# volivan239/raytracing-course-hw

Measured on AMD Instinct MI355X. Metric: Msamples/sec at 1920x1080x256spp, higher is better.
Workload: dtype f32; 1 GPU; synth_room_v1_1920x1080x256; scene=synth_room_v1 (seed 20241223), triangles=268816, emissive_triangles=4204, width=1920, height=1080, spp=256, ray_depth=6, parallelism=pixel tiles 32x32 round-robin over 1 GPU(s), bvh_nodes=265605, bvh_depth=24, light_bvh_depth=19, device_bytes=120573816

## Files before the change

raytracing-course-hw_amd/csrc/device/rt_device.h:

```cpp
#pragma once
#include <hip/hip_runtime.h>
#include "rt_types.h"

#define RT_DEV __device__ __forceinline__

namespace rtamd {
namespace dev {

struct F3 { float x, y, z; };
RT_DEV F3 f3(float x, float y, float z) { F3 r; r.x = x; r.y = y; r.z = z; return r; }
RT_DEV F3 f3(const float *p) { return f3(p[0], p[1], p[2]); }
RT_DEV F3 operator+(F3 a, F3 b) { return f3(a.x + b.x, a.y + b.y, a.z + b.z); }
RT_DEV F3 operator-(F3 a, F3 b) { return f3(a.x - b.x, a.y - b.y, a.z - b.z); }
RT_DEV F3 operator*(F3 a, F3 b) { return f3(a.x * b.x, a.y * b.y, a.z * b.z); }
RT_DEV F3 operator*(float k, F3 p) { return f3(k * p.x, k * p.y, k * p.z); }
RT_DEV F3 neg(F3 a) { return f3(-a.x, -a.y, -a.z); }
RT_DEV float dot(F3 a, F3 b) { return a.x * b.x + a.y * b.y + a.z * b.z; }
RT_DEV F3 crossr(F3 a, F3 o) { return f3(a.z * o.y - a.y * o.z, a.x * o.z - a.z * o.x, a.y * o.x - a.x * o.y); }
RT_DEV float len2(F3 a) { return dot(a, a); }
RT_DEV float len(F3 a) { return sqrtf(len2(a)); }
RT_DEV F3 normalize(F3 a) { return (1.0f / len(a)) * a; }
RT_DEV float smin(float a, float b) { return (b < a) ? b : a; }
RT_DEV float smax(float a, float b) { return (a < b) ? b : a; }

// ... 202 lines not shown
    F3 ro = o - a;
    float dn = dot(d, n);
    t = -dot(ro, n) / dn;
    if (!(t > 0 && t < RT_T_MAX)) return false;
    inside = dn > 0;
    F3 p = ro + t * d;
    float c1 = RT_MAGIC1_0 * p.x + RT_MAGIC1_1 * p.y + RT_MAGIC1_2 * p.z;
    float c2 = RT_MAGIC2_0 * p.x + RT_MAGIC2_1 * p.y + RT_MAGIC2_2 * p.z;
    float yy = (c1 * T.a2 - c2 * T.a1) / T.den;
    float xx = T.a2 == 0 ? (c1 - T.b1 * yy) / T.a1 : (c2 - T.b2 * yy) / T.a2;
    u = xx; v = yy;
    if (u < 0 || v < 0 || u + v > 1) return false;
    return true;
}

RT_DEV bool tri_test_closer(const TriIsect &T, F3 o, F3 d, float keep_t, float &t, float &u, float &v, bool &inside) {
    F3 a = f3(T.ax, T.ay, T.az), n = f3(T.nx, T.ny, T.nz);
    F3 ro = o - a;
    float dn = dot(d, n);
    t = -dot(ro, n) / dn;
    if (!(t > 0 && t < RT_T_MAX)) return false;
    if (t > keep_t) return false;
    inside = dn > 0;
    F3 p = ro + t * d;
    float c1 = RT_MAGIC1_0 * p.x + RT_MAGIC1_1 * p.y + RT_MAGIC1_2 * p.z;
    float c2 = RT_MAGIC2_0 * p.x + RT_MAGIC2_1 * p.y + RT_MAGIC2_2 * p.z;
    float yy = (c1 * T.a2 - c2 * T.a1) / T.den;
    float xx = T.a2 == 0 ? (c1 - T.b1 * yy) / T.a1 : (c2 - T.b2 * yy) / T.a2;
    u = xx; v = yy;
    if (u < 0 || v < 0 || u + v > 1) return false;
    return true;
}

RT_DEV TriIsect load_isect(const TriIsect *p) {
    const float4 *q = reinterpret_cast<const float4 *>(p);
    float4 a = q[0], b = q[1], c = q[2];
    TriIsect T;
    T.ax = a.x; T.ay = a.y; T.az = a.z; T.nx = a.w;
    T.ny = b.x; T.nz = b.y; T.a1 = b.z; T.b1 = b.w;
    T.a2 = c.x; T.b2 = c.y; T.den = c.z; T.pad = __float_as_uint(c.w);
    return T;
}

struct RayInv { F3 o, inv; };
RT_DEV RayInv make_ray_inv(F3 o, F3 d) {
    RayInv r;
    r.o = o;
    float dx = fabsf(d.x) > 1e-30f ? d.x : copysignf(1e-30f, d.x);
    float dy = fabsf(d.y) > 1e-30f ? d.y : copysignf(1e-30f, d.y);
    float dz = fabsf(d.z) > 1e-30f ? d.z : copysignf(1e-30f, d.z);
    r.inv = f3(1.0f / dx, 1.0f / dy, 1.0f / dz);
    return r;
}
RT_DEV bool slab_test(float4 lo, float4 hi, const RayInv &r, float tbest, float &tnear) {
    float t0x = (lo.x - r.o.x) * r.inv.x, t1x = (hi.x - r.o.x) * r.inv.x;
    float t0y = (lo.y - r.o.y) * r.inv.y, t1y = (hi.y - r.o.y) * r.inv.y;
    float t0z = (lo.z - r.o.z) * r.inv.z, t1z = (hi.z - r.o.z) * r.inv.z;
    float tmin = fmaxf(fmaxf(fminf(t0x, t1x), fminf(t0y, t1y)), fminf(t0z, t1z));
    float tmax = fminf(fminf(fmaxf(t0x, t1x), fmaxf(t0y, t1y)), fmaxf(t0z, t1z));
    tmin = fmaf(-fabsf(tmin), 4.8e-7f, tmin);
    tmax = fmaf(fabsf(tmax), 4.8e-7f, tmax);
    tnear = tmin;
    return (tmin <= tmax) & (tmax >= 0.f) & (tmin <= tbest);
}

typedef float rt_f2 __attribute__((ext_vector_type(2)));
struct RayGrid { float cx, cy, cz, ix, iy, iz; uint32_t sx, sy, sz; };
RT_DEV RayGrid ray_grid_idle() {
    RayGrid g;
    g.cx = 0.f; g.cy = 0.f; g.cz = 0.f; g.ix = 1.f; g.iy = 1.f; g.iz = 1.f; g.sx = 0x03020100u; g.sy = 0x03020100u; g.sz = 0x03020100u;
    return g;
}
#define RT_GRID_RAY_IDLE ray_grid_idle()
RT_DEV RayGrid make_ray_grid(const NodeGrid &G, F3 o, F3 d) {
// ... 410 lines not shown
```

raytracing-course-hw_amd/csrc/device/rt_exact.h:

```cpp
#pragma once
#include "rt_kernels_hw8.h"

namespace rtamd {
namespace dev {

#define PT_SHADE_EXACT 4
#define WF_MISS 0xFFFFFFFFu
#define WF_INSIDE_BIT 0x40000000u
#define WF_GAP_SHIFT 24
#define WF_INDEX_MASK 0x00FFFFFFu
#define WF_SAMPLE_MASK 0x01FFFFFFu
#define WF_VERIFIED_BIT 0x80000000u

template <class A>
RT_DEV void ref_closest_hit(const SceneView &S, F3 o, F3 d, A &&stack, float &best_t, float &best_u, float &best_v, uint32_t &hit) {
    best_t = RT_T_MAX; best_u = 0.f; best_v = 0.f; hit = WF_MISS;
    if (S.n_tris == 0) return;
    RefBest best = {false, RT_T_MAX};
    ref_left_first<RT_STACK_SIZE>(S.ref_nodes, o, d, stack, best, [&](uint32_t first, uint32_t last) {
        for (uint32_t i = first; i < last; i++) {
            const TriIsect T = load_isect(S.tri_isect + i);
            float t, u, v; bool in;
            if (tri_test(T, o, d, t, u, v, in) && (!best.have || t < best.t)) {
                best.have = true; best.t = t; best_u = u; best_v = v; hit = i | (in ? WF_INSIDE_BIT : 0u);
// ... 85 lines not shown
    const float window = need - fminf(fminf(ax, ay), az);
    return worst >= need && exit_ >= need && tmax - t > window;
}

RT_DEV bool pt_tripwire(const SceneView &S, F3 o, F3 d) {
    if (S.n_tripwire_groups == 0u) return false;
    const float dx = fabsf(d.x) > 1e-30f ? d.x : copysignf(1e-30f, d.x), dy = fabsf(d.y) > 1e-30f ? d.y : copysignf(1e-30f, d.y), dz = fabsf(d.z) > 1e-30f ? d.z : copysignf(1e-30f, d.z);
    RayInv r; r.o = o; r.inv = f3(pt_rcp(dx), pt_rcp(dy), pt_rcp(dz));
    const float4 *rec = reinterpret_cast<const float4 *>(S.tripwires);
    bool pierced = false;
    for (uint32_t g = 0; g < S.n_tripwire_groups; g++) {
        const float4 lo = rec[2 * g], hi = rec[2 * g + 1];
        float tn;
        if (slab_test(lo, hi, r, RT_T_MAX, tn)) {
            const uint32_t first = __float_as_uint(lo.w), count = __float_as_uint(hi.w);
            for (uint32_t m = first; m < first + count; m++) {
                const float4 mlo = rec[2 * m];
                if (slab_test(mlo, rec[2 * m + 1], r, RT_T_MAX, tn)) {
                    const uint32_t fi = __float_as_uint(mlo.w);
                    const TriIsect T = load_isect(S.tri_isect + fi);
                    float t, u, v; bool inside;
                    if (tri_test(T, o, d, t, u, v, inside)) {
                        const float4 *bx = reinterpret_cast<const float4 *>(S.tri_box) + 2 * (size_t)fi;
                        const float4 blo = bx[0], bhi = bx[1];
                        if (!pt_deep_inside(f3(blo.x, blo.y, blo.z), f3(bhi.x, bhi.y, bhi.z), o + t * d, d, t, S.box_c2)) pierced = true;
                    }
                }
            }
        }
    }
    return pierced;
}

RT_DEV bool pt_light_test(const LightRec *L, F3 x, F3 d, bool &last, uint32_t &index, float &t, float &u, float &v, bool &inside) {
    const TriIsect T = load_isect(&L->isect);
    last = (T.pad & 1u) != 0;
    index = T.pad >> 1;
    return tri_test(T, x, d, t, u, v, inside);
}
RT_DEV float pt_light_pdf_hit(const SceneView &S, const LightRec *L, F3 x, F3 d, float t, float u, float v, bool inside, bool &robust) {
    robust = true;
    const float4 *q = reinterpret_cast<const float4 *>(L) + 3;
    float4 q1 = q[1], q2 = q[2], q3 = q[3];
    float point_prob = q1.z;
    F3 n3 = f3(q1.w, q2.x, q2.y), dn1 = f3(q2.z, q2.w, q3.x), dn2 = f3(q3.y, q3.z, q3.w);
    F3 sn = n3 + u * dn1 + v * dn2;
    sn = normalize(sn);
    if (inside) sn = neg(sn);
    if (S.hw7) { const TriIsect T = load_isect(&L->isect); F3 n = f3(T.nx, T.ny, T.nz); sn = normalize(inside ? neg(n) : n); }
    F3 y = x + t * d;
    if (S.exact_boxes == 1u) {
        const float4 blo = q[4], bhi = q[5];
        robust = pt_box_robust(f3(blo.x, blo.y, blo.z), f3(bhi.x, bhi.y, bhi.z), y, d, t, S.box_c2);
    }
    return point_prob * len2(x - y) / fabsf(dot(d, sn));
}
RT_DEV float pt_light_pdf_one(const SceneView &S, const LightRec *L, F3 x, F3 d, bool &last, bool &robust, uint32_t &index) {
    TriIsect T = load_isect(&L->isect);
    last = (T.pad & 1u) != 0;
    index = T.pad >> 1;
    robust = true;
    float t, u, v; bool inside;
    if (!tri_test(T, x, d, t, u, v, inside)) return 0.f;
    const float4 *q = reinterpret_cast<const float4 *>(L) + 3;
    float4 q1 = q[1], q2 = q[2], q3 = q[3];
    float point_prob = q1.z;
    F3 n3 = f3(q1.w, q2.x, q2.y), dn1 = f3(q2.z, q2.w, q3.x), dn2 = f3(q3.y, q3.z, q3.w);
    F3 sn = n3 + u * dn1 + v * dn2;
    sn = normalize(sn);
    if (inside) sn = neg(sn);
    if (S.hw7) { F3 n = f3(T.nx, T.ny, T.nz); sn = normalize(inside ? neg(n) : n); }
    F3 y = x + t * d;
    if (S.exact_boxes == 1u) {
        const float4 blo = q[4], bhi = q[5];
        robust = pt_box_robust(f3(blo.x, blo.y, blo.z), f3(bhi.x, bhi.y, bhi.z), y, d, t, S.box_c2);
    }
    return point_prob * len2(x - y) / fabsf(dot(d, sn));
}


}
}
```

raytracing-course-hw_amd/csrc/device/rt_persistent.h:

```cpp
#pragma once
#include "rt_path_source.h"
#include "rt_pt_queue.h"

namespace rtamd {
namespace dev {

#define P8_WAVES 4
#define P8_THREADS (64 * P8_WAVES)
#define P8_PER_CU 5
#define PT_MAX_PATHS 5120
#define PT_MIN_GROUP 16
#define PT_NW (PT_MAX_PATHS / 32)
#define PT_BIT_T 1u
#define PT_BIT_L 2u
#define PT_Q_TRACE 0
#define PT_Q_LIGHT 1
#define PT_Q_SHADE 2
#define PT_Q_XLIGHT 3
#define PT_Q_XTRACE 4
#define PT_N_LIVE 5
#define PT_W_TRACE 6
#define PT_W_LIGHT 7
#define PT_GSHIFT 15
#define PT_COST_TRACE_NODE 1u
#define PT_COST_TRACE_TRI 1u
#define PT_COST_LIGHT_NODE 2u
#define PT_COST_LIGHT_TEST 2u
#define PT_COST_SHADE 14u
#define PT_DEBUG_BLOCKS 2048
#define PT_DRAINED 0xFFFFFFFEu
#define PT_T_OVERFLOW (-1.f)
#define PT_WIDE_NONE 0
#define PT_WIDE_WENT 1
#define PT_WIDE_FULL 2
RT_DEV uint32_t pt_near_key(bool entered, uint32_t key) { return entered ? key : 0xFFFFFFFFu; }
RT_DEV void pt_order(uint32_t &ka, uint32_t &ca, uint32_t &kb, uint32_t &cb) {
    const bool s = kb < ka;
    const uint32_t k = s ? kb : ka, c = s ? cb : ca;
    kb = s ? ka : kb; cb = s ? ca : cb;
    ka = k; ca = c;
}
RT_DEV int pt_wide_step_nearest(const GpuNode4Q *nodes, const RayGrid &ray, float cull_t, uint32_t (*stack)[64], int lane, int &sp, int cap, uint32_t &cur) {
    const uint4 *q = reinterpret_cast<const uint4 *>(nodes + cur);
    const uint4 b0 = q[0], b1 = q[1], b2 = q[2], b3 = q[3];
    uint32_t k0, k1, k2, k3;
    const bool h0 = slab_enter_q(b0, ray, cull_t, k0), h1 = slab_enter_q(b1, ray, cull_t, k1);
    const bool h2 = slab_enter_q(b2, ray, cull_t, k2), h3 = slab_enter_q(b3, ray, cull_t, k3);
    k0 = pt_near_key(h0, k0); k1 = pt_near_key(h1, k1); k2 = pt_near_key(h2, k2); k3 = pt_near_key(h3, k3);
    uint32_t c0 = b0.w, c1 = b1.w, c2 = b2.w, c3 = b3.w;
    pt_order(k0, c0, k1, c1); pt_order(k2, c2, k3, c3); pt_order(k0, c0, k2, c2); pt_order(k1, c1, k3, c3); pt_order(k1, c1, k2, c2);
    const int nh = (int)h0 + (int)h1 + (int)h2 + (int)h3;
    if (nh == 0) return PT_WIDE_NONE;
    if (sp + nh - 1 > cap) return PT_WIDE_FULL;
    if (nh > 3) stack[sp++][lane] = c3;
    if (nh > 2) stack[sp++][lane] = c2;
    if (nh > 1) stack[sp++][lane] = c1;
    cur = c0;
    return PT_WIDE_WENT;
}
RT_DEV void pt_wide_enter_all(const GpuNode4Q *nodes, uint32_t cur, const RayGrid &ray, uint4 &b0, uint4 &b1, uint4 &b2, uint4 &b3,
                              bool &h0, bool &h1, bool &h2, bool &h3) {
    const uint4 *q = reinterpret_cast<const uint4 *>(nodes + cur);
    b0 = q[0]; b1 = q[1]; b2 = q[2]; b3 = q[3];
    h0 = slab_test_q(b0, ray); h1 = slab_test_q(b1, ray); h2 = slab_test_q(b2, ray); h3 = slab_test_q(b3, ray);
}
RT_DEV int pt_wide_step_all(const GpuNode4Q *nodes, const RayGrid &ray, uint32_t (*stack)[64], int lane, int &sp, int cap, uint32_t &cur) {
    uint4 b0, b1, b2, b3;
    bool h0, h1, h2, h3;
    pt_wide_enter_all(nodes, cur, ray, b0, b1, b2, b3, h0, h1, h2, h3);
    const int nh = (int)h0 + (int)h1 + (int)h2 + (int)h3;
    if (nh == 0) return PT_WIDE_NONE;
    if (sp + nh - 1 > cap) return PT_WIDE_FULL;
    const int first = h0 ? 0 : h1 ? 1 : h2 ? 2 : 3;
    if (h3 && first != 3) stack[sp++][lane] = b3.w;
    if (h2 && first < 2) stack[sp++][lane] = b2.w;
    if (h1 && first < 1) stack[sp++][lane] = b1.w;
    cur = first == 0 ? b0.w : first == 1 ? b1.w : first == 2 ? b2.w : b3.w;
    return PT_WIDE_WENT;
}
#define PT_LIGHT_SETTLE 1
template <int LEVELS>
RT_DEV int pt_light_reach(const SceneView &S, const RayGrid &ray, int &steps) {
    uint4 b[4];
    bool h[4];
    pt_wide_enter_all(S.light_walk_nodes4, 0u, ray, b[0], b[1], b[2], b[3], h[0], h[1], h[2], h[3]);
    steps = 1;
    if (!(h[0] | h[1] | h[2] | h[3])) return 0;
    if (LEVELS < 2) return 2;
    for (int c = 0; c < 4; c++) {
        if (!h[c]) continue;
        if (b[c].w & RT_LEAF_BIT) return 2;
        uint4 g0, g1, g2, g3;
        bool e0, e1, e2, e3;
        pt_wide_enter_all(S.light_walk_nodes4, b[c].w, ray, g0, g1, g2, g3, e0, e1, e2, e3);
        steps++;
        if (e0 | e1 | e2 | e3) return 2;
    }
    return 1;
}
#define PT_EXACT_BATCH 16

struct PtShared {
    uint32_t stack[P8_WAVES][P8_STACK][64];
    uint32_t need[5][PT_NW];
    uint32_t pending[PT_NW * 2];
    uint32_t groups[PT_MAX_PATHS / PT_MIN_GROUP];
    uint32_t cost[PT_MAX_PATHS / PT_MIN_GROUP];
    int cnt[16];
};
static_assert(PT_EXACT_BATCH * RT_STACK_SIZE <= P8_STACK * 64, "the exact role's stacks must fit the wave's LDS stack area");
static_assert(sizeof(PtShared) <= (128 / P8_PER_CU) * 1280, "P8_PER_CU workgroups per CU: the CU's 128 LDS granules of 1,280 bytes shared evenly");

struct PtParams {
    uint32_t n_groups;
    uint32_t group_shift;
    const uint32_t *group_ofs, *group_ids;
    uint32_t *group_cost;
    uint32_t resume;
    int refill, leaf_batch;
    int shade_min;
    int shade_thr0, shade_thr_step;
    int cost_t, cost_l;
    uint32_t front_first;
    int prio;
    unsigned long long deadline_ticks;
    unsigned long long *counters;
    unsigned long long *debug;
// ... 134 lines not shown
                if (went == PT_WIDE_NONE) {
                    if (sp != 0) cur = stack[--sp][lane];
                    else if (pend != RT_EMPTY_LEAF) cur = PT_DRAINED;
                    else end_walk();
                } else if (went == PT_WIDE_FULL) {
                    w.full();
                    pend = RT_EMPTY_LEAF; pend2 = RT_EMPTY_LEAF; pend3 = RT_EMPTY_LEAF;
                    end_walk();
                }
            }
        }
        clk.lap(prof.t_part[K][1]);
        const bool at_leaf = active && pend != RT_EMPTY_LEAF;
        if (COUNT) { prof.leaf_iters[K]++; prof.leaf_lane_iters[K] += __popcll(pt_ballot(at_leaf)); }
        if (at_leaf) {
            uint32_t i = pend & ~RT_LEAF_BIT, more = pend2, more2 = pend3;
            typename WK::Leaf lf;
            for (;;) {
                const bool last = w.test(i, sp, lf);
                if (COUNT) n_tris++;
                steps += WK::COST_TEST;
                if (!last) i++;
                else if (more == RT_EMPTY_LEAF) break;
                else { i = more & ~RT_LEAF_BIT; more = more2; more2 = RT_EMPTY_LEAF; }
            }
            const bool over = w.leaves_done(lf, sp);
            pend = RT_EMPTY_LEAF; pend2 = RT_EMPTY_LEAF; pend3 = RT_EMPTY_LEAF;
            if (cur == PT_DRAINED || over) end_walk();
        }
        clk.lap(prof.t_part[K][2]);
    }
}

template <class T> RT_DEV const T *pt_own_pointer(const T *p) { asm volatile("" : "+s"(p)); return p; }
struct PtTraceWalk {
    typedef PtTraceQueue Queue;
    static constexpr uint32_t COST_NODE = PT_COST_TRACE_NODE, COST_TEST = PT_COST_TRACE_TRI;
    const SceneView &S; const WfView &W; PtShared &sh; const PtParams &P; uint32_t (*stack)[64];
    const GpuNode4Q *nodes = pt_own_pointer(S.nodes4);
    const int lane = threadIdx.x & 63;
    F3 o = f3(0.f, 0.f, 0.f), d = f3(0.f, 0.f, 1.f);
    RayGrid ray = RT_GRID_RAY_IDLE;
    uint32_t hit = WF_MISS;
    float best_t = RT_T_MAX, best_u = 0.f, best_v = 0.f;
    float cull_t = RT_T_MAX, t2 = 2.f * RT_T_MAX, h_ray = 0.f;
    struct Leaf {};
    RT_DEV void begin(uint32_t slot) {
        const float4 *r = wf_rec(W, slot);
        float4 q0 = r[0], q1 = r[1];
        o = f3(q0.x, q0.y, q0.z); d = f3(q0.w, q1.x, q1.y);
        ray = make_ray_grid(S.grid, o, d);
        h_ray = S.exact_boxes ? pt_look_behind_abs(d, S.box_c2x) : 0.f;
        hit = WF_MISS; best_t = RT_T_MAX; cull_t = RT_T_MAX; t2 = 2.f * RT_T_MAX; best_u = 0.f; best_v = 0.f;
    }
    RT_DEV int step(uint32_t &cur, int &sp) { return pt_wide_step_nearest(nodes, ray, cull_t, stack, lane, sp, P8_STACK, cur); }
    RT_DEV void full() { best_t = PT_T_OVERFLOW; best_u = 0.f; best_v = 0.f; hit = 0u; t2 = PT_T_OVERFLOW; }
    RT_DEV bool test(uint32_t i, int, Leaf &) {
        TriIsect T = load_isect(S.tri_walk + i);
        float t, u, v; bool inside;
        const uint32_t fi = T.pad >> 1;
        if (tri_test_closer(T, o, d, cull_t, t, u, v, inside)) {
            const uint32_t best_i = hit & WF_INDEX_MASK;
            if (t < best_t || (t == best_t && fi < best_i)) {
                t2 = fminf(t2, best_t);
                best_t = t; best_u = u; best_v = v; hit = fi | (inside ? WF_INSIDE_BIT : 0u);
                cull_t = t + fmaxf(S.cull_k * t, h_ray);
            } else t2 = fminf(t2, t);
        }
        return (T.pad & 1u) != 0u;
    }
    RT_DEV bool leaves_done(Leaf &, int) { return false; }
    RT_DEV uint32_t end(uint32_t l, uint32_t slot, uint32_t steps) {
        wf_rec(W, slot)[2] = make_float4(best_t, best_u, best_v, __uint_as_float(S.exact_boxes && hit != WF_MISS ? hit | pt_gap_code(best_t, t2) : hit));
        pt_book_cost(sh, P, l, steps);
        return l;
    }
};

template <bool COUNT> struct PtLightWalk {
    typedef PtLightQueue<PT_Q_XLIGHT> Queue;
    static constexpr uint32_t COST_NODE = PT_COST_LIGHT_NODE, COST_TEST = PT_COST_LIGHT_TEST;
    const SceneView &S; const WfView &W; PtShared &sh; const PtParams &P; uint32_t (*stack)[64]; PtProf &prof;
    const GpuNode4Q *nodes = pt_own_pointer(S.light_walk_nodes4);
    const LightRec *lights = pt_own_pointer(S.lights_walk);
    const int lane = threadIdx.x & 63;
    bool overflow = false;
    int k = 0;
    F3 o = f3(0.f, 0.f, 0.f), d = f3(0.f, 0.f, 1.f);
    RayGrid ray = RT_GRID_RAY_IDLE;
    struct Leaf { bool held = false; uint32_t h_i = 0u, h_li = 0u; float h_t = 0.f, h_u = 0.f, h_v = 0.f; bool h_in = false; };
    RT_DEV void begin(uint32_t slot) {
        const float4 *r = wf_rec(W, slot);
        float4 q0 = r[0], q1 = r[1];
        o = f3(q0.x, q0.y, q0.z); d = f3(q0.w, q1.x, q1.y);
        ray = make_ray_grid(S.grid, o, d);
        k = 0; overflow = false;
    }
    RT_DEV int step(uint32_t &cur, int &sp) { return pt_wide_step_all(nodes, ray, stack, lane, sp, P8_STACK - 2 * k - 1, cur); }
    RT_DEV void full() { overflow = true; }
    RT_DEV void take(Leaf &lf, int sp) {
        bool robust;
        const float term = pt_light_pdf_hit(S, lights + lf.h_i, o, d, lf.h_t, lf.h_u, lf.h_v, lf.h_in, robust);
        if (COUNT && term != 0.f) prof.light_hits++;
        if (term != 0.f) {
            if (!robust || k >= WF_MAX_LIGHT_HITS || sp + 2 * k + 2 >= P8_STACK) overflow = true;
            else {
                int j = k;
                while (j > 0 && stack[P8_STACK - 1 - 2 * (j - 1)][lane] > lf.h_li) {
                    stack[P8_STACK - 1 - 2 * j][lane] = stack[P8_STACK - 1 - 2 * (j - 1)][lane];
                    stack[P8_STACK - 2 - 2 * j][lane] = stack[P8_STACK - 2 - 2 * (j - 1)][lane];
                    j--;
                }
                stack[P8_STACK - 1 - 2 * j][lane] = lf.h_li; stack[P8_STACK - 2 - 2 * j][lane] = __float_as_uint(term); k++;
            }
        }
        lf.held = false;
    }
    RT_DEV bool test(uint32_t i, int sp, Leaf &lf) {
        bool last, inside; uint32_t li; float t, u, v;
        if (COUNT) prof.light_tests++;
        if (pt_light_test(lights + i, o, d, last, li, t, u, v, inside)) {
            if (lf.held) take(lf, sp);
            lf.held = true; lf.h_i = i; lf.h_li = li; lf.h_t = t; lf.h_u = u; lf.h_v = v; lf.h_in = inside;
        }
        return last;
    }
    RT_DEV bool leaves_done(Leaf &lf, int sp) { if (lf.held) take(lf, sp); return false; }
    RT_DEV uint32_t end(uint32_t l, uint32_t slot, uint32_t steps) {
        pt_book_cost(sh, P, l, steps);
        if (overflow) return l | 0x80000000u;
        float v = 0.f;
        if (k == 1) v = __uint_as_float(stack[P8_STACK - 2][lane]);
        else if (k == 2) v = __uint_as_float(stack[P8_STACK - 2][lane]) + __uint_as_float(stack[P8_STACK - 4][lane]);
        else if (k > 2) {
            const uint32_t nl = S.n_lights;
            for (int j = 1; j < k; j++) {
                uint32_t a0 = stack[P8_STACK - 1 - 2 * (j - 1)][lane], b0 = stack[P8_STACK - 1 - 2 * j][lane];
                uint32_t len = b0 - a0;
                uint32_t lv = 31u - (uint32_t)__clz((int)len);
                uint16_t m0 = S.light_sep[(size_t)lv * nl + a0], m1 = S.light_sep[(size_t)lv * nl + (b0 - (1u << lv))];
                stack[j - 1][lane] = m0 < m1 ? m0 : m1;
            }
            for (int n = k; n > 1; n--) {
                int best = 1;
                uint32_t bd = stack[0][lane];
                for (int i = 2; i < n; i++) { uint32_t di = stack[i - 1][lane]; if (di > bd) { bd = di; best = i; } }
                float merged = __uint_as_float(stack[P8_STACK - 2 - 2 * (best - 1)][lane]) + __uint_as_float(stack[P8_STACK - 2 - 2 * best][lane]);
                stack[P8_STACK - 2 - 2 * (best - 1)][lane] = __float_as_uint(merged);
                for (int i = best; i < n - 1; i++) {
                    stack[P8_STACK - 2 - 2 * i][lane] = stack[P8_STACK - 2 - 2 * (i + 1)][lane];
                    stack[i - 1][lane] = stack[i][lane];
                }
            }
            v = __uint_as_float(stack[P8_STACK - 2][lane]);
// ... 366 lines not shown
                r[3] = make_float4(0.f, 0.f, 0.f, __uint_as_float(wf_pack(0, false, (uint32_t)R.samples)));
                if (P.counters && pt_source_counts(R, gslot)) atomicAdd(&P.counters[CNT_SRC_NO_PATH], 1ull);
                return false;
            }
        } else {
            if (R.sample_seeds) wf_sample_seed(R, rng, gslot, x, y, 0u);
            wf_camera_ray(S, R, rng, x, y, o, d);
        }
        r[0] = make_float4(o.x, o.y, o.z, d.x);
        r[1] = make_float4(d.y, d.z, __uint_as_float(rng.x), rng.saved);
        r[2] = make_float4(0.f, 0.f, 0.f, 0.f);
        r[3] = make_float4(sum.x, sum.y, sum.z, __uint_as_float(wf_pack(0, rng.has_saved, R.accum ? (uint32_t)R.sample_first : 0u)));
        return true;
    }
    RT_DEV uint32_t resumed_sample(uint32_t slot) { return (__float_as_uint(reinterpret_cast<const float *>(wf_rec(W, slot) + 3)[3]) >> 6) & WF_SAMPLE_MASK; }
    RT_DEV bool seed_wire(uint32_t slot) {
        if constexpr ((FEAT & WF_FEAT_SOURCE) != 0) {
            const float4 *nr = wf_rec(W, slot);
            const float4 n0 = nr[0], n1 = nr[1];
            return pt_source_exact(S, f3(n0.x, n0.y, n0.z), f3(n0.w, n1.x, n1.y));
        }
        if (!S.n_tripwire_groups) return false;
        const float4 *nr = wf_rec(W, slot);
        const float4 n0 = nr[0], n1 = nr[1];
        return pt_tripwire(S, f3(n0.x, n0.y, n0.z), f3(n0.w, n1.x, n1.y));
    }
    RT_DEV bool rare(PtWave &wv) {
        const bool queued = pt_count(&sh.cnt[PT_Q_XLIGHT]) + pt_count(&sh.cnt[PT_Q_XTRACE]) > 0;
        if (queued) pt_exact_batch(S, W, sh, wv, &stack[0][0], n_xlight, n_xtrace);
        return queued;
    }
    RT_DEV PtShaded shade(uint32_t got, uint32_t &n_light, unsigned long long &n_nodes, PtProf &prof) {
        const uint32_t lane = threadIdx.x & 63u;
        int todo = 0;
        bool discarded = false;
        if (COUNT && P.trace_buf && got != PT_NONE) {
            const uint32_t tslot = pt_slot(sh, got);
            int tx, ty; bool tin; size_t toi;
            wf_slot_to_pixel(R, tslot + W.slot_base, tx, ty, tin, toi);
            if (tin && ty * R.width + tx == P.trace_pixel) {
                const float4 *tr = wf_rec(W, tslot);
                const uint32_t k = atomicAdd(reinterpret_cast<uint32_t *>(P.trace_buf), 1u);
                if (4u * k + 5u <= P.trace_cap) for (int q = 0; q < 4; q++) P.trace_buf[1 + 4 * k + q] = tr[q];
            }
        }
        PtShadeLap<COUNT> lp;
        if (got != PT_NONE) { PtPark pk; pk.p = (PtLdsWord)&stack[0][lane]; todo = pt_shade_lean<FEAT>(S, R, W, pt_slot(sh, got), pk, discarded, lp); }
        if constexpr (COUNT) {
            for (int k = 0; k < 5; k++) {
                const unsigned long long m = pt_ballot(lp.d[k] != 0u);
                if (m) { prof.t_shade[k] += (uint32_t)__builtin_amdgcn_readlane((int)lp.d[k], __builtin_ctzll(m)); prof.shade_lanes[k] += __popcll(m); }
            }
            prof.shade_last += __popcll(pt_ballot(lp.last));
        }
        n_discarded += __popcll(pt_ballot(discarded));
        const bool next = got != PT_NONE && todo != PT_SHADE_EXACT && (todo & WF_NEXT_TRACE), with_light = next && (todo & WF_NEXT_LIGHT);
        bool wire = false;
        bool settled = false;
        int settle_steps = 0;
        if (next && (S.n_tripwire_groups || ((COUNT || PT_LIGHT_SETTLE) && with_light))) {
            const float4 *nr = wf_rec(W, pt_slot(sh, got));
            const float4 n0 = nr[0], n1 = nr[1];
            const F3 o = f3(n0.x, n0.y, n0.z), d = f3(n0.w, n1.x, n1.y);
            if (S.n_tripwire_groups) wire = pt_tripwire(S, o, d);
            if ((COUNT || PT_LIGHT_SETTLE) && with_light) {
                const int reach = pt_light_reach<COUNT ? 2 : PT_LIGHT_SETTLE>(S, make_ray_grid(S.grid, o, d), settle_steps);
                if (COUNT) { prof.light_reach[0] += reach == 0; prof.light_reach[1] += reach == 1; }
                settled = reach < PT_LIGHT_SETTLE;
                if (settled) {
                    const int depth = (int)(__float_as_uint(reinterpret_cast<const float *>(nr + 3)[3]) & 15u);
                    float *pdf = reinterpret_cast<float *>(wf_entry(W, pt_slot(sh, got), depth)) + 3;
                    *pdf = *pdf + 0.f / S.n_lights_f;
                }
            }
        }
        if constexpr ((FEAT & WF_FEAT_SOURCE) != 0) {
            if (next && !wire) {
                const float4 *nr = wf_rec(W, pt_slot(sh, got));
                if ((__float_as_uint(reinterpret_cast<const float *>(nr + 3)[3]) & (15u | WF_PENDING_BIT)) == 0u) {
                    const float4 n0 = nr[0], n1 = nr[1];
                    wire = pt_source_exact(S, f3(n0.x, n0.y, n0.z), f3(n0.w, n1.x, n1.y));
                }
            }
        }
        n_light += __popcll(pt_ballot(settled));
        if (COUNT && settled) n_nodes += (unsigned long long)settle_steps;
        PtShaded s;
        s.trace = next;
        s.light = with_light && !settled;
        s.xtrace = (got != PT_NONE && todo == PT_SHADE_EXACT) || wire;
        s.done = got != PT_NONE && (todo == 0 || todo == WF_PARKED);
        if (got != PT_NONE && todo != PT_SHADE_EXACT) s.cost = (uint32_t)PT_COST_SHADE + (settled ? PT_COST_LIGHT_NODE * (uint32_t)settle_steps : 0u);
        return s;
    }
    RT_DEV void flush(uint32_t lane, const PtProf &prof) {
        if (lane == 0) {
            if (n_discarded) atomicAdd(&P.counters[CNT_DISCARDED], (unsigned long long)n_discarded);
            if (n_xtrace) atomicAdd(&P.counters[CNT_EXACT_CLOSEST], (unsigned long long)n_xtrace);
            if (n_xlight) atomicAdd(&P.counters[CNT_EXACT_LIGHT], (unsigned long long)n_xlight);
        }
        if (!COUNT) return;
        atomicAdd(&P.counters[CNT_P8_LIGHT_HITS], prof.light_hits); atomicAdd(&P.counters[CNT_P8_LIGHT_TESTS], prof.light_tests);
        atomicAdd(&P.counters[CNT_P8_LIGHT_REACH], prof.light_reach[0]); atomicAdd(&P.counters[CNT_P8_LIGHT_REACH + 1], prof.light_reach[1]);
        if (lane == 0) {
            atomicAdd(&P.counters[CNT_P8_WALK_ITERS], prof.iters[0]); atomicAdd(&P.counters[CNT_P8_WALK_ITERS + 1], prof.lane_iters[0]);
            atomicAdd(&P.counters[CNT_P8_WALK_ITERS + 2], prof.iters[1]); atomicAdd(&P.counters[CNT_P8_WALK_ITERS + 3], prof.lane_iters[1]);
            atomicAdd(&P.counters[CNT_P8_STINTS], prof.stints); atomicAdd(&P.counters[CNT_P8_SHADE_BATCHES], prof.shade_batches); atomicAdd(&P.counters[CNT_P8_SHADE_ITEMS], prof.shade_items);
            for (int k = 0; k < 3; k++) atomicAdd(&P.counters[CNT_P8_HANDOFF_TIME + k], prof.t_sub[0][k]);
            atomicAdd(&P.counters[CNT_P8_HANDOFFS], prof.refills[0]);
            for (int k = 0; k < 5; k++) { atomicAdd(&P.counters[CNT_P8_SHADE_TIME + k], prof.t_shade[k]); atomicAdd(&P.counters[CNT_P8_SHADE_LANES + k], prof.shade_lanes[k]); }
            atomicAdd(&P.counters[CNT_P8_SHADE_LAST], prof.shade_last);
// ... 22 lines not shown
```

raytracing-course-hw_amd/csrc/device/rt_types.h:

```cpp
#pragma once
#include <stdint.h>

namespace rtamd {

#define RT_MAX_DEPTH 16
#define RT_STACK_SIZE 64
#define P8_STACK 24

enum CounterSlot {
    CNT_CLOSEST = 0,
    CNT_LIGHT = 1,
    CNT_NODE_VISITS = 2,
    CNT_TRI_TESTS = 3,
    CNT_WF_NODE_ITERS = 4,
    CNT_WF_LEAF_PHASES = 5,
    CNT_WF_LEAF_LANES = 6,
    CNT_WF_REFILLS = 7,
    CNT_WF_LANE_NODES = 8,
    CNT_WF_LANE_TRIS = 9,
    CNT_DISCARDED = 10,
    CNT_WF_SLOW_LIGHT = 11,
    CNT_P6_EXACT_LIGHT = 11,
    CNT_EXACT_CLOSEST = 12,
    CNT_EXACT_LIGHT = 13,
// ... 39 lines not shown
#define RT_GRID_BORDER 4
struct NodeGrid { float lo[3], step[3], istep[3]; };

struct TriIsect {
    float ax, ay, az;
    float nx, ny, nz;
    float a1, b1;
    float a2, b2;
    float den;
    uint32_t pad;
};
static_assert(sizeof(TriIsect) == 48, "TriIsect must be 48 bytes");

struct TriShade {
    float n3[3], dn1[3], dn2[3];
    float t3[3], dt1[3], dt2[3];
    float uv3[2], duv1[2], duv2[2];
    float tanw;
    uint32_t material;
    uint32_t orig;
    uint32_t pad;
};
static_assert(sizeof(TriShade) == 112, "TriShade must be 112 bytes");

struct LightRec {
    TriIsect isect;
    float b[3], c[3];
    float point_prob;
    float n3[3], dn1[3], dn2[3];
    float box_lo[3], pad0;
    float box_hi[3], pad1;
};
static_assert(sizeof(LightRec) == 48 + 64 + 32, "LightRec must be 144 bytes");

struct GpuRefNode {
    float mn[3]; uint32_t left;
    float mx[3]; uint32_t right;
    uint32_t first, last, pad0, pad1;
};
static_assert(sizeof(GpuRefNode) == 48, "GpuRefNode must be 48 bytes");

struct GpuMaterial {
    float base_color[3]; float metallic_factor;
    float emission[3];   float roughness_factor;
    int32_t base_color_tex, emissive_tex, metallic_roughness_tex, normal_tex;
};
static_assert(sizeof(GpuMaterial) == 48, "GpuMaterial must be 48 bytes");

struct GpuImage {
    uint64_t offset;
    int32_t width, height;
};

struct SceneView {
    const GpuNode *nodes;
    const TriIsect *tri_isect;
    float cull_k;
    const TriIsect *tri_walk;
    const TriShade *tri_shade;
    const GpuNode *light_nodes;
    const LightRec *lights;
    const GpuNode *light_walk_nodes;
    const float *tripwires;
    uint32_t n_tripwire_groups;
    const GpuNode4Q *nodes4, *light_walk_nodes4;
    NodeGrid grid;
    const LightRec *lights_walk;
    const uint16_t *light_sep;
    const GpuMaterial *materials;
    const GpuImage *images;
    const uint8_t *texels;
    const float *srgb_lut;
    const GpuRefNode *ref_nodes, *ref_light_nodes;
    const float *tri_box;
    float box_c2;
    float box_c2x;
    uint32_t exact_boxes;
    uint32_t n_tris, n_lights, n_components;
    float n_lights_f, n_components_f;
    uint32_t n_nodes;
    uint32_t last_level_emission_only;
    uint32_t hw7;
    int32_t env_image;
    float cam_pos[3], cam_right[3], cam_up[3], cam_fwd[3];
    float bg[3];
    float tan_fov_y;
};

struct RenderView {
    int32_t width, height, samples, ray_depth;
    int32_t sample_stop;
    int32_t tile_w, tile_h, tiles_x, tiles_y;
    int32_t shard_index, shard_count;
    uint32_t n_shard_tiles;
    float tan_fov_x;
    float inv_samples;
    float *out_rgb;
    uint8_t *out_rgb8;
    uint32_t *work_counter;
    unsigned long long *counters;
// ... 18 lines not shown
```

raytracing-course-hw_amd/csrc/rtamd_scene.hip:

```cpp
#include <hip/hip_runtime.h>
#include <cmath>
#include <cstdio>
#include <cstdlib>
#include <cstring>
#include <memory>
#include <string>
#include <vector>
#include "../../include/rtamd.h"
#include "host/host_scene.h"
#include "host/png.h"
#include "host/scene_prep.h"
#include "host/shared_prep.h"
#include "host/device_build.h"
#include "host/knobs.h"
#include "host/rt_scene.h"
#include "device/rt_node_grid.h"

namespace rtamd {
static thread_local std::string g_last_error;
void set_error(const std::string &msg) { g_last_error = msg; }
}
using namespace rtamd;

namespace {
// ... 183 lines not shown
        const uint32_t n = desc->n_triangles;
        uint64_t scratch = 0;
        OwnedDev d_walk_box;
        if (!P.walk_box.empty()) d_walk_box.p = upload(P.walk_box, scratch);
        const DeviceTree t = build_leaf_ordered(s.get(), d_walk_box.p ? (const float *)d_walk_box.p : V.tri_box, V.tri_isect, n, P.box_pad, P8_STACK,
                                                11, true, V.tri_walk);
        V.nodes = t.nodes;
        up.bytes += (uint64_t)t.n_nodes * sizeof(GpuNode) + (uint64_t)n * sizeof(TriIsect);
        bvh_depth = t.depth;
        n_nodes = t.n_nodes;
        s->info.bvh_build_ms = t.build_ms; s->info.bvh_on_device = 1;
    } else {
        V.nodes = up(P.nodes);
        V.tri_walk = V.tri_isect;
    }
    if (P.bvh_depth > RT_STACK_SIZE - 2)
        return fail(RT_ERR_LIMIT, "the reference's scene BVH is deeper than the exact walk's stack (" + std::to_string(P.bvh_depth) + ")");
    if (bvh_depth > RT_STACK_SIZE - 2 || P.light_bvh_depth > RT_STACK_SIZE - 2)
        return fail(RT_ERR_LIMIT, "scene BVH deeper than the kernel's traversal stack (" + std::to_string(bvh_depth) + "/" +
                                      std::to_string(P.light_bvh_depth) + ")");
    V.light_nodes = up(P.light_nodes);
    V.light_sep = up(P.light_sep);
    upload_ref_trees(V, P, up);
    set_triangle_view(V, *desc, P, 2u);
    V.box_c2x *= (float)env_float("RTAMD_C2X_SCALE", 1.0);
    V.exact_boxes = (env_flag("RTAMD_NO_EXACT_BOXES") || fast_build) ? 0u : 1u;
    if (env_flag("RTAMD_DIAG_LOOKBEHIND_ONLY")) V.exact_boxes = 2u;
    V.n_tripwire_groups = (V.exact_boxes != 1u || env_flag("RTAMD_NO_TRIPWIRES")) ? 0u : P.n_tripwire_groups;
    V.tripwires = V.n_tripwire_groups ? up(P.tripwires) : nullptr;
    V.lights = up(P.lights);
    uint32_t n_light_walk_nodes = 0;
    {
        const uint32_t nl = (uint32_t)P.lights.size();
        std::vector<LightRec> tagged = P.lights;
        for (uint32_t i = 0; i < nl; i++) tagged[i].isect.pad = (i << 1) | (tagged[i].isect.pad ? 1u : 0u);
        if (nl >= 64 && !env_flag("RTAMD_HOST_LIGHT_BVH")) {
            uint64_t scratch = 0;
            OwnedDev d_tagged(upload(tagged, up.bytes));
            OwnedDev d_lbox(upload(P.light_walk_box, scratch));
            const DeviceTree lt = build_leaf_ordered(s.get(), (const float *)d_lbox.p, (const LightRec *)d_tagged.p, nl, P.box_pad, 16,
                                                     11, true, V.lights_walk);
            V.light_walk_nodes = lt.nodes;
            up.bytes += (uint64_t)lt.n_nodes * sizeof(GpuNode);
            s->light_walk_depth = lt.depth;
            n_light_walk_nodes = lt.n_nodes;
        } else {
            V.light_walk_nodes = V.light_nodes;
            n_light_walk_nodes = (uint32_t)P.light_nodes.size();
            V.lights_walk = up(tagged);
            s->light_walk_depth = P.light_bvh_depth;
        }
    }
    V.materials = up(P.materials);
    V.images = up(P.images);
    V.texels = up(P.texels);
    V.srgb_lut = up(std::vector<float>(P.srgb_lut, P.srgb_lut + 256));
    V.n_nodes = n_nodes;
    V.last_level_emission_only = 1;
    for (uint32_t i = 0; i < desc->n_materials; i++) {
        const rt_material &m = desc->materials[i];
        if (!(m.metallic_factor >= 0 && m.metallic_factor <= 1 && m.base_color[0] >= 0 && m.base_color[1] >= 0 && m.base_color[2] >= 0))
            V.last_level_emission_only = 0;
    }
    if (env_flag("RTAMD_NO_LAST_LEVEL_SHORTCUT")) V.last_level_emission_only = 0;
    V.env_image = P.env_image;
    make_walk_nodes(s.get(), V.cam_pos, V.nodes, n_nodes, V.light_walk_nodes, n_light_walk_nodes, n_light_walk_nodes != 0,
                    V.grid, V.nodes4, V.light_walk_nodes4, up.bytes);
    report_trees(s.get(), desc, P, V.n_lights, n_nodes, bvh_depth);
    return finish_scene(s, out, up.bytes, t0, t1);
}

}

int rtamd::scene_create_shared(const rt_scene_desc *desc, rt_scene **out, rtamd::SharedPrep *shared) {
    if (!desc || !out) return fail(RT_ERR_INVALID_ARG, "rt_scene_create: null argument");
    if (desc->struct_size != sizeof(rt_scene_desc)) return fail(RT_ERR_INVALID_ARG, "rt_scene_create: struct_size mismatch (ABI skew)");
    *out = nullptr;
    int ndev = 0;
    if (hipGetDeviceCount(&ndev) != hipSuccess || ndev == 0)
        return fail(RT_ERR_NO_DEVICE, "rt_scene_create: no HIP device available (this library has no CPU fallback)");
    return guarded("", [&]() -> int {
        std::unique_ptr<rt_scene> s(new rt_scene());
        HIP_CHECK(hipGetDevice(&s->device));
        hipDeviceProp_t prop;
        HIP_CHECK(hipGetDeviceProperties(&prop, s->device));
        s->n_cus = prop.multiProcessorCount > 0 ? prop.multiProcessorCount : 256;
        const double t0 = now_ms();
        if (desc->n_triangles == 0 && (desc->n_primitives > 0 || (desc->camera.fov_x != 0.f && desc->camera.fov_y == 0.f))) return create_txt(desc, s, out, t0);
        if (desc->n_triangles && !desc->normals) return create_hw6(desc, s, out, t0);
        return create_hw8(desc, s, out, t0, shared);
    });
}

extern "C" {

const char *rt_last_error(void) { return g_last_error.c_str(); }

int rt_scene_create(const rt_scene_desc *desc, rt_scene **out) { return rtamd::scene_create_shared(desc, out, nullptr); }
// ... 104 lines not shown
```

Before: 514.2 Msamples/s.

## Split light records into hot and cold arrays and use 32-bit global offsets

Splits the 144-byte light record into a 48-byte intersection array and a 96-byte remainder array, so light tests in the walker read only the compact hot part. Node, triangle and light loads now use address_space(1) pointers with 32-bit byte offsets (umul24), and the light BVH root is read through a constant-address-space pointer. Both aim to cut address arithmetic and wasted memory traffic. In exchange it adds a scene-size limit check for the 32-bit offsets and an extra device-to-device split copy at scene build time.

```diff
diff --git a/raytracing-course-hw_amd/csrc/device/rt_device.h b/raytracing-course-hw_amd/csrc/device/rt_device.h
--- a/raytracing-course-hw_amd/csrc/device/rt_device.h
+++ b/raytracing-course-hw_amd/csrc/device/rt_device.h
@@ -258,14 +258,32 @@
     return true;
 }
 
-RT_DEV TriIsect load_isect(const TriIsect *p) {
-    const float4 *q = reinterpret_cast<const float4 *>(p);
-    float4 a = q[0], b = q[1], c = q[2];
+RT_DEV TriIsect isect_of(float4 a, float4 b, float4 c) {
     TriIsect T;
     T.ax = a.x; T.ay = a.y; T.az = a.z; T.nx = a.w;
     T.ny = b.x; T.nz = b.y; T.a1 = b.z; T.b1 = b.w;
     T.a2 = c.x; T.b2 = c.y; T.den = c.z; T.pad = __float_as_uint(c.w);
     return T;
+}
+RT_DEV TriIsect load_isect(const TriIsect *p) {
+    const float4 *q = reinterpret_cast<const float4 *>(p);
+    const float4 a = q[0], b = q[1], c = q[2];
+    return isect_of(a, b, c);
+}
+
+#define RT_GLOBAL __attribute__((address_space(1)))
+struct GlobalBytes {
+    const RT_GLOBAL char *base;
+    typedef uint32_t Word4 __attribute__((ext_vector_type(4)));
+    RT_DEV uint4 u4(uint32_t ofs, uint32_t k = 0u) const { const Word4 w = reinterpret_cast<const RT_GLOBAL Word4 *>(base + ofs)[k]; return make_uint4(w.x, w.y, w.z, w.w); }
+    RT_DEV float4 f4(uint32_t ofs, uint32_t k = 0u) const { const uint4 w = u4(ofs, k); return make_float4(__uint_as_float(w.x), __uint_as_float(w.y), __uint_as_float(w.z), __uint_as_float(w.w)); }
+};
+RT_DEV GlobalBytes global_bytes(const void *p) { return GlobalBytes{(const RT_GLOBAL char *)p}; }
+RT_DEV GlobalBytes global_bytes_own(const void *p) { asm volatile("" : "+s"(p)); return global_bytes(p); }
+RT_DEV uint32_t record_ofs(uint32_t i, uint32_t stride) { return __umul24(i, stride); }
+RT_DEV TriIsect load_isect(const GlobalBytes &g, uint32_t ofs) {
+    const float4 a = g.f4(ofs, 0u), b = g.f4(ofs, 1u), c = g.f4(ofs, 2u);
+    return isect_of(a, b, c);
 }
 
 struct RayInv { F3 o, inv; };
diff --git a/raytracing-course-hw_amd/csrc/device/rt_exact.h b/raytracing-course-hw_amd/csrc/device/rt_exact.h
--- a/raytracing-course-hw_amd/csrc/device/rt_exact.h
+++ b/raytracing-course-hw_amd/csrc/device/rt_exact.h
@@ -141,25 +141,26 @@
     return pierced;
 }
 
-RT_DEV bool pt_light_test(const LightRec *L, F3 x, F3 d, bool &last, uint32_t &index, float &t, float &u, float &v, bool &inside) {
-    const TriIsect T = load_isect(&L->isect);
+RT_DEV bool pt_light_test(const GlobalBytes &tests, uint32_t i, F3 x, F3 d, bool &last, uint32_t &index, float &t, float &u, float &v, bool &inside) {
+    const TriIsect T = load_isect(tests, record_ofs(i, (uint32_t)sizeof(TriIsect)));
     last = (T.pad & 1u) != 0;
     index = T.pad >> 1;
     return tri_test(T, x, d, t, u, v, inside);
 }
-RT_DEV float pt_light_pdf_hit(const SceneView &S, const LightRec *L, F3 x, F3 d, float t, float u, float v, bool inside, bool &robust) {
+RT_DEV float pt_light_pdf_hit(const SceneView &S, const GlobalBytes &tests, const GlobalBytes &rests, uint32_t i, F3 x, F3 d, float t, float u, float v, bool inside, bool &robust) {
     robust = true;
-    const float4 *q = reinterpret_cast<const float4 *>(L) + 3;
-    float4 q1 = q[1], q2 = q[2], q3 = q[3];
+    uint32_t q = record_ofs(i, (uint32_t)sizeof(LightRest));
+    const float4 q1 = rests.f4(q, 1u), q2 = rests.f4(q, 2u), q3 = rests.f4(q, 3u);
     float point_prob = q1.z;
     F3 n3 = f3(q1.w, q2.x, q2.y), dn1 = f3(q2.z, q2.w, q3.x), dn2 = f3(q3.y, q3.z, q3.w);
     F3 sn = n3 + u * dn1 + v * dn2;
     sn = normalize(sn);
     if (inside) sn = neg(sn);
-    if (S.hw7) { const TriIsect T = load_isect(&L->isect); F3 n = f3(T.nx, T.ny, T.nz); sn = normalize(inside ? neg(n) : n); }
+    if (S.hw7) { const TriIsect T = load_isect(tests, record_ofs(i, (uint32_t)sizeof(TriIsect))); F3 n = f3(T.nx, T.ny, T.nz); sn = normalize(inside ? neg(n) : n); }
     F3 y = x + t * d;
     if (S.exact_boxes == 1u) {
-        const float4 blo = q[4], bhi = q[5];
+        asm volatile("" : "+v"(q));
+        const float4 blo = rests.f4(q, 4u), bhi = rests.f4(q, 5u);
         robust = pt_box_robust(f3(blo.x, blo.y, blo.z), f3(bhi.x, bhi.y, bhi.z), y, d, t, S.box_c2);
     }
     return point_prob * len2(x - y) / fabsf(dot(d, sn));
diff --git a/raytracing-course-hw_amd/csrc/device/rt_persistent.h b/raytracing-course-hw_amd/csrc/device/rt_persistent.h
--- a/raytracing-course-hw_amd/csrc/device/rt_persistent.h
+++ b/raytracing-course-hw_amd/csrc/device/rt_persistent.h
@@ -40,9 +40,18 @@
     kb = s ? ka : kb; cb = s ? ca : cb;
     ka = k; ca = c;
 }
-RT_DEV int pt_wide_step_nearest(const GpuNode4Q *nodes, const RayGrid &ray, float cull_t, uint32_t (*stack)[64], int lane, int &sp, int cap, uint32_t &cur) {
+RT_DEV void pt_node_records(const GpuNode4Q *nodes, uint32_t cur, uint4 &b0, uint4 &b1, uint4 &b2, uint4 &b3) {
     const uint4 *q = reinterpret_cast<const uint4 *>(nodes + cur);
-    const uint4 b0 = q[0], b1 = q[1], b2 = q[2], b3 = q[3];
+    b0 = q[0]; b1 = q[1]; b2 = q[2]; b3 = q[3];
+}
+RT_DEV void pt_node_records(const GlobalBytes nodes, uint32_t cur, uint4 &b0, uint4 &b1, uint4 &b2, uint4 &b3) {
+    const uint32_t ofs = cur << 6;
+    b0 = nodes.u4(ofs, 0u); b1 = nodes.u4(ofs, 1u); b2 = nodes.u4(ofs, 2u); b3 = nodes.u4(ofs, 3u);
+}
+template <class NODES>
+RT_DEV int pt_wide_step_nearest(const NODES nodes, const RayGrid &ray, float cull_t, uint32_t (*stack)[64], int lane, int &sp, int cap, uint32_t &cur) {
+    uint4 b0, b1, b2, b3;
+    pt_node_records(nodes, cur, b0, b1, b2, b3);
     uint32_t k0, k1, k2, k3;
     const bool h0 = slab_enter_q(b0, ray, cull_t, k0), h1 = slab_enter_q(b1, ray, cull_t, k1);
     const bool h2 = slab_enter_q(b2, ray, cull_t, k2), h3 = slab_enter_q(b3, ray, cull_t, k3);
@@ -58,13 +67,21 @@
     cur = c0;
     return PT_WIDE_WENT;
 }
-RT_DEV void pt_wide_enter_all(const GpuNode4Q *nodes, uint32_t cur, const RayGrid &ray, uint4 &b0, uint4 &b1, uint4 &b2, uint4 &b3,
+template <class NODES>
+RT_DEV void pt_wide_enter_all(const NODES nodes, uint32_t cur, const RayGrid &ray, uint4 &b0, uint4 &b1, uint4 &b2, uint4 &b3,
                               bool &h0, bool &h1, bool &h2, bool &h3) {
-    const uint4 *q = reinterpret_cast<const uint4 *>(nodes + cur);
-    b0 = q[0]; b1 = q[1]; b2 = q[2]; b3 = q[3];
+    pt_node_records(nodes, cur, b0, b1, b2, b3);
     h0 = slab_test_q(b0, ray); h1 = slab_test_q(b1, ray); h2 = slab_test_q(b2, ray); h3 = slab_test_q(b3, ray);
 }
-RT_DEV int pt_wide_step_all(const GpuNode4Q *nodes, const RayGrid &ray, uint32_t (*stack)[64], int lane, int &sp, int cap, uint32_t &cur) {
+struct PtRootNode { const GpuNode4Q *nodes; };
+RT_DEV void pt_node_records(const PtRootNode root, uint32_t, uint4 &b0, uint4 &b1, uint4 &b2, uint4 &b3) {
+    typedef const __attribute__((address_space(4))) GlobalBytes::Word4 *Q;
+    const Q q = (Q)root.nodes;
+    const GlobalBytes::Word4 w0 = q[0], w1 = q[1], w2 = q[2], w3 = q[3];
+    b0 = make_uint4(w0.x, w0.y, w0.z, w0.w); b1 = make_uint4(w1.x, w1.y, w1.z, w1.w); b2 = make_uint4(w2.x, w2.y, w2.z, w2.w); b3 = make_uint4(w3.x, w3.y, w3.z, w3.w);
+}
+template <class NODES>
+RT_DEV int pt_wide_step_all(const NODES nodes, const RayGrid &ray, uint32_t (*stack)[64], int lane, int &sp, int cap, uint32_t &cur) {
     uint4 b0, b1, b2, b3;
     bool h0, h1, h2, h3;
     pt_wide_enter_all(nodes, cur, ray, b0, b1, b2, b3, h0, h1, h2, h3);
@@ -83,7 +100,8 @@
 RT_DEV int pt_light_reach(const SceneView &S, const RayGrid &ray, int &steps) {
     uint4 b[4];
     bool h[4];
-    pt_wide_enter_all(S.light_walk_nodes4, 0u, ray, b[0], b[1], b[2], b[3], h[0], h[1], h[2], h[3]);
+    const GlobalBytes nodes = global_bytes(S.light_walk_nodes4);
+    pt_wide_enter_all(PtRootNode{S.light_walk_nodes4}, 0u, ray, b[0], b[1], b[2], b[3], h[0], h[1], h[2], h[3]);
     steps = 1;
     if (!(h[0] | h[1] | h[2] | h[3])) return 0;
     if (LEVELS < 2) return 2;
@@ -92,7 +110,7 @@
         if (b[c].w & RT_LEAF_BIT) return 2;
         uint4 g0, g1, g2, g3;
         bool e0, e1, e2, e3;
-        pt_wide_enter_all(S.light_walk_nodes4, b[c].w, ray, g0, g1, g2, g3, e0, e1, e2, e3);
+        pt_wide_enter_all(nodes, b[c].w, ray, g0, g1, g2, g3, e0, e1, e2, e3);
         steps++;
         if (e0 | e1 | e2 | e3) return 2;
     }
@@ -293,12 +311,11 @@
     }
 }
 
-template <class T> RT_DEV const T *pt_own_pointer(const T *p) { asm volatile("" : "+s"(p)); return p; }
 struct PtTraceWalk {
     typedef PtTraceQueue Queue;
     static constexpr uint32_t COST_NODE = PT_COST_TRACE_NODE, COST_TEST = PT_COST_TRACE_TRI;
     const SceneView &S; const WfView &W; PtShared &sh; const PtParams &P; uint32_t (*stack)[64];
-    const GpuNode4Q *nodes = pt_own_pointer(S.nodes4);
+    const GlobalBytes nodes = global_bytes_own(S.nodes4), tris = global_bytes(S.tri_walk);
     const int lane = threadIdx.x & 63;
     F3 o = f3(0.f, 0.f, 0.f), d = f3(0.f, 0.f, 1.f);
     RayGrid ray = RT_GRID_RAY_IDLE;
@@ -317,7 +334,7 @@
     RT_DEV int step(uint32_t &cur, int &sp) { return pt_wide_step_nearest(nodes, ray, cull_t, stack, lane, sp, P8_STACK, cur); }
     RT_DEV void full() { best_t = PT_T_OVERFLOW; best_u = 0.f; best_v = 0.f; hit = 0u; t2 = PT_T_OVERFLOW; }
     RT_DEV bool test(uint32_t i, int, Leaf &) {
-        TriIsect T = load_isect(S.tri_walk + i);
+        TriIsect T = load_isect(tris, record_ofs(i, (uint32_t)sizeof(TriIsect)));
         float t, u, v; bool inside;
         const uint32_t fi = T.pad >> 1;
         if (tri_test_closer(T, o, d, cull_t, t, u, v, inside)) {
@@ -342,8 +359,7 @@
     typedef PtLightQueue<PT_Q_XLIGHT> Queue;
     static constexpr uint32_t COST_NODE = PT_COST_LIGHT_NODE, COST_TEST = PT_COST_LIGHT_TEST;
     const SceneView &S; const WfView &W; PtShared &sh; const PtParams &P; uint32_t (*stack)[64]; PtProf &prof;
-    const GpuNode4Q *nodes = pt_own_pointer(S.light_walk_nodes4);
-    const LightRec *lights = pt_own_pointer(S.lights_walk);
+    const GlobalBytes nodes = global_bytes_own(S.light_walk_nodes4), tests = global_bytes_own(S.lights_walk_test), rests = global_bytes(S.lights_walk_rest);
     const int lane = threadIdx.x & 63;
     bool overflow = false;
     int k = 0;
@@ -361,7 +377,7 @@
     RT_DEV void full() { overflow = true; }
     RT_DEV void take(Leaf &lf, int sp) {
         bool robust;
-        const float term = pt_light_pdf_hit(S, lights + lf.h_i, o, d, lf.h_t, lf.h_u, lf.h_v, lf.h_in, robust);
+        const float term = pt_light_pdf_hit(S, tests, rests, lf.h_i, o, d, lf.h_t, lf.h_u, lf.h_v, lf.h_in, robust);
         if (COUNT && term != 0.f) prof.light_hits++;
         if (term != 0.f) {
             if (!robust || k >= WF_MAX_LIGHT_HITS || sp + 2 * k + 2 >= P8_STACK) overflow = true;
@@ -380,7 +396,7 @@
     RT_DEV bool test(uint32_t i, int sp, Leaf &lf) {
         bool last, inside; uint32_t li; float t, u, v;
         if (COUNT) prof.light_tests++;
-        if (pt_light_test(lights + i, o, d, last, li, t, u, v, inside)) {
+        if (pt_light_test(tests, i, o, d, last, li, t, u, v, inside)) {
             if (lf.held) take(lf, sp);
             lf.held = true; lf.h_i = i; lf.h_li = li; lf.h_t = t; lf.h_u = u; lf.h_v = v; lf.h_in = inside;
         }
@@ -813,10 +829,11 @@
     }
     RT_DEV PtShaded shade(uint32_t got, uint32_t &n_light, unsigned long long &n_nodes, PtProf &prof) {
         const uint32_t lane = threadIdx.x & 63u;
+        const uint32_t slot = got != PT_NONE ? pt_slot(sh, got) : 0u;
         int todo = 0;
         bool discarded = false;
         if (COUNT && P.trace_buf && got != PT_NONE) {
-            const uint32_t tslot = pt_slot(sh, got);
+            const uint32_t tslot = slot;
             int tx, ty; bool tin; size_t toi;
             wf_slot_to_pixel(R, tslot + W.slot_base, tx, ty, tin, toi);
             if (tin && ty * R.width + tx == P.trace_pixel) {
@@ -826,7 +843,7 @@
             }
         }
         PtShadeLap<COUNT> lp;
-        if (got != PT_NONE) { PtPark pk; pk.p = (PtLdsWord)&stack[0][lane]; todo = pt_shade_lean<FEAT>(S, R, W, pt_slot(sh, got), pk, discarded, lp); }
+        if (got != PT_NONE) { PtPark pk; pk.p = (PtLdsWord)&stack[0][lane]; todo = pt_shade_lean<FEAT>(S, R, W, slot, pk, discarded, lp); }
         if constexpr (COUNT) {
             for (int k = 0; k < 5; k++) {
                 const unsigned long long m = pt_ballot(lp.d[k] != 0u);
@@ -840,7 +857,7 @@
         bool settled = false;
         int settle_steps = 0;
         if (next && (S.n_tripwire_groups || ((COUNT || PT_LIGHT_SETTLE) && with_light))) {
-            const float4 *nr = wf_rec(W, pt_slot(sh, got));
+            const float4 *nr = wf_rec(W, slot);
             const float4 n0 = nr[0], n1 = nr[1];
             const F3 o = f3(n0.x, n0.y, n0.z), d = f3(n0.w, n1.x, n1.y);
             if (S.n_tripwire_groups) wire = pt_tripwire(S, o, d);
@@ -850,14 +867,14 @@
                 settled = reach < PT_LIGHT_SETTLE;
                 if (settled) {
                     const int depth = (int)(__float_as_uint(reinterpret_cast<const float *>(nr + 3)[3]) & 15u);
-                    float *pdf = reinterpret_cast<float *>(wf_entry(W, pt_slot(sh, got), depth)) + 3;
+                    float *pdf = reinterpret_cast<float *>(wf_entry(W, slot, depth)) + 3;
                     *pdf = *pdf + 0.f / S.n_lights_f;
                 }
             }
         }
         if constexpr ((FEAT & WF_FEAT_SOURCE) != 0) {
             if (next && !wire) {
-                const float4 *nr = wf_rec(W, pt_slot(sh, got));
+                const float4 *nr = wf_rec(W, slot);
                 if ((__float_as_uint(reinterpret_cast<const float *>(nr + 3)[3]) & (15u | WF_PENDING_BIT)) == 0u) {
                     const float4 n0 = nr[0], n1 = nr[1];
                     wire = pt_source_exact(S, f3(n0.x, n0.y, n0.z), f3(n0.w, n1.x, n1.y));
diff --git a/raytracing-course-hw_amd/csrc/device/rt_types.h b/raytracing-course-hw_amd/csrc/device/rt_types.h
--- a/raytracing-course-hw_amd/csrc/device/rt_types.h
+++ b/raytracing-course-hw_amd/csrc/device/rt_types.h
@@ -95,6 +95,21 @@
     float box_hi[3], pad1;
 };
 static_assert(sizeof(LightRec) == 48 + 64 + 32, "LightRec must be 144 bytes");
+struct LightRest {
+    float b[3], c[3];
+    float point_prob;
+    float n3[3], dn1[3], dn2[3];
+    float box_lo[3], pad0;
+    float box_hi[3], pad1;
+};
+static_assert(sizeof(LightRest) == sizeof(LightRec) - sizeof(TriIsect) && sizeof(LightRest) == 96, "LightRest must be the 96 bytes of a LightRec after its TriIsect");
+
+#define RT_WALK_MAX_RECORDS (1u << 24)
+inline bool walk_arrays_fit(uint64_t n_tris, uint64_t n_lights, uint64_t n_nodes, uint64_t n_light_nodes) {
+    const uint64_t lim = 1ull << 32;
+    return n_tris <= RT_WALK_MAX_RECORDS && n_lights <= RT_WALK_MAX_RECORDS && n_tris * sizeof(TriIsect) < lim && n_lights * sizeof(LightRest) < lim &&
+           n_nodes * sizeof(GpuNode4Q) < lim && n_light_nodes * sizeof(GpuNode4Q) < lim;
+}
 
 struct GpuRefNode {
     float mn[3]; uint32_t left;
@@ -128,7 +143,8 @@
     uint32_t n_tripwire_groups;
     const GpuNode4Q *nodes4, *light_walk_nodes4;
     NodeGrid grid;
-    const LightRec *lights_walk;
+    const TriIsect *lights_walk_test;
+    const LightRest *lights_walk_rest;
     const uint16_t *light_sep;
     const GpuMaterial *materials;
     const GpuImage *images;
diff --git a/raytracing-course-hw_amd/csrc/rtamd_scene.hip b/raytracing-course-hw_amd/csrc/rtamd_scene.hip
--- a/raytracing-course-hw_amd/csrc/rtamd_scene.hip
+++ b/raytracing-course-hw_amd/csrc/rtamd_scene.hip
@@ -239,6 +239,7 @@
     uint32_t n_light_walk_nodes = 0;
     {
         const uint32_t nl = (uint32_t)P.lights.size();
+        const LightRec *ordered = nullptr;
         std::vector<LightRec> tagged = P.lights;
         for (uint32_t i = 0; i < nl; i++) tagged[i].isect.pad = (i << 1) | (tagged[i].isect.pad ? 1u : 0u);
         if (nl >= 64 && !env_flag("RTAMD_HOST_LIGHT_BVH")) {
@@ -246,7 +247,7 @@
             OwnedDev d_tagged(upload(tagged, up.bytes));
             OwnedDev d_lbox(upload(P.light_walk_box, scratch));
             const DeviceTree lt = build_leaf_ordered(s.get(), (const float *)d_lbox.p, (const LightRec *)d_tagged.p, nl, P.box_pad, 16,
-                                                     11, true, V.lights_walk);
+                                                     11, true, ordered);
             V.light_walk_nodes = lt.nodes;
             up.bytes += (uint64_t)lt.n_nodes * sizeof(GpuNode);
             s->light_walk_depth = lt.depth;
@@ -254,9 +255,20 @@
         } else {
             V.light_walk_nodes = V.light_nodes;
             n_light_walk_nodes = (uint32_t)P.light_nodes.size();
-            V.lights_walk = up(tagged);
+            ordered = up(tagged);
             s->light_walk_depth = P.light_bvh_depth;
         }
+        OwnedDev whole(s->allocations.back());
+        s->allocations.pop_back();
+        const size_t n_rec = nl ? nl : 1u;
+        char *pair = nullptr;
+        HIP_CHECK(hipMalloc((void **)&pair, n_rec * sizeof(LightRec)));
+        s->allocations.push_back(pair);
+        char *rest = pair + n_rec * sizeof(TriIsect);
+        HIP_CHECK(hipMemcpy2D(pair, sizeof(TriIsect), ordered, sizeof(LightRec), sizeof(TriIsect), n_rec, hipMemcpyDeviceToDevice));
+        HIP_CHECK(hipMemcpy2D(rest, sizeof(LightRest), (const char *)ordered + sizeof(TriIsect), sizeof(LightRec), sizeof(LightRest), n_rec, hipMemcpyDeviceToDevice));
+        V.lights_walk_test = (const TriIsect *)pair;
+        V.lights_walk_rest = (const LightRest *)rest;
     }
     V.materials = up(P.materials);
     V.images = up(P.images);
@@ -271,6 +283,8 @@
     }
     if (env_flag("RTAMD_NO_LAST_LEVEL_SHORTCUT")) V.last_level_emission_only = 0;
     V.env_image = P.env_image;
+    if (!walk_arrays_fit(desc->n_triangles, V.n_lights, n_nodes, n_light_walk_nodes))
+        return fail(RT_ERR_LIMIT, "the scene's triangles, lights or tree nodes do not fit the walkers' 32-bit offsets (2^24 records, 4 GiB per array)");
     make_walk_nodes(s.get(), V.cam_pos, V.nodes, n_nodes, V.light_walk_nodes, n_light_walk_nodes, n_light_walk_nodes != 0,
                     V.grid, V.nodes4, V.light_walk_nodes4, up.bytes);
     report_trees(s.get(), desc, P, V.n_lights, n_nodes, bvh_depth);
```

New measurement: 540.4 Msamples/s, median of 6. 1.05x the previous value.
